# zzuiekongning/MGDT-YOLO

Hardware: AMD Instinct MI355X
Metric: images/sec @640x640 bs=32 per GPU, detection forward + NMS (whole job: 1 GPU(s)) (higher is better)
Workload: dtype bf16; 1 GPU; mspa_c2f_gd_yolov8-n (MSPA-C2f + GD neck + Detect, nc=80) 640x640 inference, batch 32/GPU: forward + decode + NMS(conf 0.25, iou 0.7), hipGraph replay, 4 batches in flight (one captured graph per resident batch, replayed round-robin on 4 streams); global_batch=32, parallelism=replicas x1 (batch-sharded, no data-path collective), rccl_ranks=1, input=bfloat16 NCHW images, 8 different batches resident in HBM (600 MiB) cycled, detections_last_step=9600, weights=seeded random init (no checkpoints offline), batches_in_flight=4

## Files before the change

### include/mgdt.h

```cpp
#ifndef MGDT_H
#define MGDT_H
#include <stddef.h>
#include <stdint.h>

#ifdef __cplusplus
extern "C" {
#endif

typedef void* mgdt_stream;

typedef enum { MGDT_OK = 0, MGDT_BAD_SHAPE = -1, MGDT_BAD_DTYPE = -2, MGDT_LAUNCH_FAIL = -3, MGDT_BAD_ARG = -4,
               MGDT_WORKSPACE = -5 } mgdt_status;
typedef enum { MGDT_F32 = 0, MGDT_BF16 = 1, MGDT_U8 = 2  } mgdt_dtype;
typedef enum { MGDT_ACT_NONE = 0, MGDT_ACT_SILU = 1, MGDT_ACT_RELU = 2, MGDT_ACT_GELU = 3 } mgdt_act;

typedef struct {
  void* p;
  int32_t n, h, w, c;
  int64_t sn, sh, sw, sc;
} mgdt_view;

const char* mgdt_last_error(void);
const char* mgdt_version(void);

size_t mgdt_conv_packed_bytes(int cin, int cout, int k, int dtype);
int mgdt_conv_pack(const float* w_oihw, const float* conv_bias, const float* bn_gamma, const float* bn_beta,
                   const float* bn_mean, const float* bn_var, float bn_eps, int cin, int cout, int k, int dtype,
                   void* packed_out, float* bias_out, mgdt_stream s);
int mgdt_conv_pack_dgrad(const float* w_oihw, int cin, int cout, int k, int phase, int dtype, void* packed_out, float* bias_out, mgdt_stream s);
typedef struct mgdt_pack_desc {
  const float* w; const float* conv_bias; const float* bn_gamma; const float* bn_beta; const float* bn_mean; const float* bn_var;
  float bn_eps; int32_t cin, cout, k, dtype, mode;
  void* packed; float* bias_out;
} mgdt_pack_desc;
int mgdt_conv_pack_batch(const mgdt_pack_desc* descs, int n, mgdt_stream s);

int mgdt_conv2d_fwd(const mgdt_view* x, const mgdt_view* x2, const float* in_scale, const float* in_shift,
                    const void* packed_w, const float* bias, int k, int stride, int act, const mgdt_view* r1,
                    const mgdt_view* r2, const mgdt_view* y, int dtype, mgdt_stream s);
size_t mgdt_conv_packed_bytes_fp8(int cin, int cout, int k);
int mgdt_conv_pack_fp8(const float* w_oihw, const float* conv_bias, const float* bn_gamma, const float* bn_beta, const float* bn_mean,
                       const float* bn_var, float bn_eps, int cin, int cout, int k, float x_qscale, void* packed_out, float* bias_out,
                       float* oscale_out, mgdt_stream s);
int mgdt_conv2d_fp8_fwd(const mgdt_view* x, const mgdt_view* x2, const float* in_scale, const float* in_shift, const void* packed_w,
                        const float* bias, const float* oscale, float x_qscale, int k, int stride, int act, const mgdt_view* r1,
                        const mgdt_view* r2, const mgdt_view* y, mgdt_stream s);
enum { MGDT_ROUTE_X2 = 1, MGDT_ROUTE_IN_SCALE = 2, MGDT_ROUTE_IN_SHIFT = 4, MGDT_ROUTE_R1 = 8, MGDT_ROUTE_R2 = 16, MGDT_ROUTE_FP8 = 32 };
enum { MGDT_ROUTE_IGEMM = 0, MGDT_ROUTE_LDS3X3 = 1 };
typedef struct {
  int32_t family, nchunks, waves, lds_bytes;
  int32_t NT, MT, D, extra, nseg, seg_chunks, gx, gy, numTiles, ragged;
  int32_t NBW, tile_rows, ncg, nwg, ntiles;
} mgdt_conv_route;
int mgdt_conv2d_route(const mgdt_view* x, const mgdt_view* y, int k, int stride, int dtype, int flags, int act, mgdt_conv_route* out);
int mgdt_conv2d_phase_fwd(const mgdt_view* x, const void* packed_w, const float* bias, int phase, const mgdt_view* r1, const mgdt_view* r2,
                          const mgdt_view* y, int dtype, mgdt_stream s);

size_t mgdt_cnx_mlp_packed_bytes(int c, int dtype);
int mgdt_cnx_mlp_pack(const float* w1, const float* b1, const float* w2, const float* b2, int c, void* packed, int dtype, mgdt_stream s);
size_t mgdt_cnx_mlp_workspace_bytes(int n, int h, int w, int c);
int mgdt_cnx_mlp_fwd(const mgdt_view* t, const mgdt_view* res, const void* packed, const float* gamma, const float* beta, void* ws,
                     const mgdt_view* y, int dtype, mgdt_stream s);

int mgdt_cnx_block_supported(int n, int h, int w, int c, int dtype);
size_t mgdt_cnx_block_workspace_bytes(int n, int h, int w, int c);
int mgdt_cnx_block_geometry(int h, int w, int c, int* out);
int mgdt_cnx_block_fwd(const mgdt_view* x, const float* dw_w49c, const float* dw_b, const float* ln_w, const float* ln_b, float eps, const void* packed,
                       const float* gamma, const float* beta, const void* tail_w, const float* tail_b, int tail_act, void* ws, size_t ws_bytes,
                       const mgdt_view* y, int dtype, mgdt_stream s);

size_t mgdt_stem2_packed_bytes(void);
int mgdt_stem2_pack(const float* w_folded, void* packed, mgdt_stream s);
int mgdt_stem2_fwd(const mgdt_view* x, int x_dtype, const void* packed0, const float* bias0, const void* packed1, const float* bias1,
                   const mgdt_view* y, mgdt_stream s);
int mgdt_stem2_geometry(int n, int h, int w, int cu_count, int* out);
int mgdt_stem2_route(const mgdt_view* x, int x_dtype, const mgdt_view* y, int cu_count, int* out);

int mgdt_detect_tail_supported(int c2, int c3, int nc, int reg_max, int dtype);
int mgdt_detect_tail_fwd(const mgdt_view* tb, const mgdt_view* tc, const void* wb, const float* bb, const void* wc, const float* bc, int nc,
                         float stride, int a_off, int a_total, const mgdt_view* feat, float* y, unsigned long long* best_keys,
                         const void* wb3, const float* bb3, mgdt_stream s);
int mgdt_detect_tail_aug_fwd(const mgdt_view* tb, const mgdt_view* tc, const void* wb, const float* bb, const void* wc, const float* bc, int nc,
                             float stride, int a_off, int a_total, const mgdt_view* feat, float* y, unsigned long long* best_keys,
                             const void* wb3, const float* bb3, float aug_scale, int aug_flip, float aug_img_w, mgdt_stream s);

// ... 251 lines not shown
```

### mgdt_yolo_amd/_lib.py

```python
import ctypes as C
import os

_HERE = os.path.dirname(os.path.abspath(__file__))
LIB_PATH = os.environ.get('MGDT_LIB') or os.path.join(_HERE, 'csrc', 'libmgdt_hip.so')

F32, BF16 = 0, 1
ACT_NONE, ACT_SILU, ACT_RELU, ACT_GELU = 0, 1, 2, 3
SPR_SPLITS = 16
GRN_SPLITS = 8


class View(C.Structure):
    _fields_ = [('p', C.c_void_p), ('n', C.c_int32), ('h', C.c_int32), ('w', C.c_int32), ('c', C.c_int32),
                ('sn', C.c_int64), ('sh', C.c_int64), ('sw', C.c_int64), ('sc', C.c_int64)]


VP = C.POINTER(View)
_vp, _i, _f, _sz, _l = C.c_void_p, C.c_int, C.c_float, C.c_size_t, C.c_long

class PackDesc(C.Structure):
    _fields_ = [('w', C.c_void_p), ('conv_bias', C.c_void_p), ('bn_gamma', C.c_void_p), ('bn_beta', C.c_void_p), ('bn_mean', C.c_void_p), ('bn_var', C.c_void_p),
                ('bn_eps', C.c_float), ('cin', C.c_int32), ('cout', C.c_int32), ('k', C.c_int32), ('dtype', C.c_int32), ('mode', C.c_int32),
                ('packed', C.c_void_p), ('bias_out', C.c_void_p)]


class WgradFinalDesc(C.Structure):
    _fields_ = [('partial', C.c_void_p), ('dw', C.c_void_p), ('n', C.c_long), ('nsplit', C.c_int32), ('accumulate', C.c_int32)]


class ConvRoute(C.Structure):
    _fields_ = [(n, C.c_int32) for n in ('family', 'nchunks', 'waves', 'lds_bytes', 'NT', 'MT', 'D', 'extra', 'nseg', 'seg_chunks', 'gx', 'gy', 'numTiles',
                                         'ragged', 'NBW', 'tile_rows', 'ncg', 'nwg', 'ntiles')]


ROUTE_X2, ROUTE_IN_SCALE, ROUTE_IN_SHIFT, ROUTE_R1, ROUTE_R2, ROUTE_FP8 = 1, 2, 4, 8, 16, 32
ROUTE_IGEMM, ROUTE_LDS3X3 = 0, 1
DIRECT_STEM, DIRECT_GENERIC, DIRECT_REFUSED = 0, 1, 2

PROTOTYPES = {
    'mgdt_last_error': (C.c_char_p, []),
    'mgdt_version': (C.c_char_p, []),
    'mgdt_conv_packed_bytes': (_sz, [_i, _i, _i, _i]),
    'mgdt_conv_pack': (_i, [_vp, _vp, _vp, _vp, _vp, _vp, _f, _i, _i, _i, _i, _vp, _vp, _vp]),
    'mgdt_conv2d_fwd': (_i, [VP, VP, _vp, _vp, _vp, _vp, _i, _i, _i, VP, VP, VP, _i, _vp]),
    'mgdt_conv_packed_bytes_fp8': (_sz, [_i, _i, _i]),
    'mgdt_conv_pack_fp8': (_i, [_vp, _vp, _vp, _vp, _vp, _vp, _f, _i, _i, _i, _f, _vp, _vp, _vp, _vp]),
    'mgdt_conv2d_fp8_fwd': (_i, [VP, VP, _vp, _vp, _vp, _vp, _vp, _f, _i, _i, _i, VP, VP, VP, _vp]),
    'mgdt_conv2d_route': (_i, [VP, VP, _i, _i, _i, _i, _i, C.POINTER(ConvRoute)]),
    'mgdt_conv_pack_batch': (_i, [_vp, _i, _vp]),
    'mgdt_conv2d_phase_fwd': (_i, [VP, _vp, _vp, _i, VP, VP, VP, _i, _vp]),
    'mgdt_conv_wgrad_splits': (_i, [_i, _i, _i]),
    'mgdt_wgrad_final_batch': (_i, [_vp, _i, _vp]),
    'mgdt_conv_pack_dgrad': (_i, [_vp, _i, _i, _i, _i, _i, _vp, _vp, _vp]),
    'mgdt_conv_pack_direct': (_i, [_vp, _vp, _vp, _vp, _vp, _vp, _f, _i, _i, _i, _vp, _vp, _vp]),
    'mgdt_conv2d_direct_fwd': (_i, [VP, _i, _vp, _vp, _i, _i, _i, _i, VP, _i, _vp]),
    'mgdt_conv2d_direct_route': (_i, [VP, _i, VP, _i, _i, _i, _i, C.POINTER(C.c_int)]),
    'mgdt_spr_pool_fwd': (_i, [VP, _vp, _i, _vp]),
    'mgdt_spr_attn_fwd': (_i, [_vp, _vp, _vp, _vp, _vp, _i, _i, _i, _i, _i, _i, _vp, _vp]),
    'mgdt_scale_channels_fwd': (_i, [VP, _vp, VP, _i, _vp]),
    'mgdt_sppf_pool_fwd': (_i, [VP, VP, VP, VP, _i, _vp]),
    'mgdt_adaptive_avgpool_fwd': (_i, [VP, VP, _i, _vp]),
    'mgdt_bilinear_fwd': (_i, [VP, VP, _i, _vp]),
    'mgdt_nearest_fwd': (_i, [VP, VP, _i, _vp]),
    'mgdt_copy_fwd': (_i, [VP, _i, VP, _i, _vp]),
    'mgdt_image_pad4_fwd': (_i, [VP, _i, VP, _i, _vp]),
    'mgdt_dwconv7_ln_fwd': (_i, [VP, _vp, _vp, _vp, _vp, _f, VP, _i, _vp]),
    'mgdt_cnx_mlp_packed_bytes': (_sz, [_i, _i]),
    'mgdt_cnx_mlp_pack': (_i, [_vp, _vp, _vp, _vp, _i, _vp, _i, _vp]),
    'mgdt_cnx_mlp_workspace_bytes': (_sz, [_i, _i, _i, _i]),
# ... 152 lines not shown
```

### mgdt_yolo_amd/csrc/common.h

```cpp
#pragma once
#include <atomic>
#include <hip/hip_runtime.h>
#include <stdint.h>
#include <stdio.h>
#include <string.h>

#include "../../include/mgdt.h"

typedef __bf16 bf16;
typedef __attribute__((ext_vector_type(8))) __bf16 bf16x8;
typedef __attribute__((ext_vector_type(4))) __bf16 bf16x4;
typedef __attribute__((ext_vector_type(4))) float f32x4;

#define MGDT_WAVE 64
#define POSE_MAX_NK 240

void mgdt_set_error(const char* fmt, ...);
#define MGDT_FAIL(code, ...)        \
  do {                              \
    mgdt_set_error(__VA_ARGS__);    \
    return (code);                  \
  } while (0)
#define MGDT_CHECK_LAUNCH(name)                                                   \
  do {                                                                            \
    hipError_t e_ = hipGetLastError();                                            \
    if (e_ != hipSuccess) MGDT_FAIL(MGDT_LAUNCH_FAIL, "%s: %s", name, hipGetErrorString(e_)); \
  } while (0)

static inline bool view_ok(const mgdt_view* v) { return v && v->p && v->n > 0 && v->h > 0 && v->w > 0 && v->c > 0; }
static inline bool view_nhwc(const mgdt_view* v) { return v->sc == 1; }
static inline int cdiv(long a, long b) { return (int)((a + b - 1) / b); }
static inline size_t dtype_size(int dt) { return dt == MGDT_BF16 ? 2 : 4; }

struct C3Plan { int NBW, MT, waves, ncg, nwg, tiles_x, tiles_per_img, ntiles, XP; size_t lds; long extx, exty; };

template <typename T> __device__ __forceinline__ float ldf(const T* p);
template <> __device__ __forceinline__ float ldf<float>(const float* p) { return *p; }
template <> __device__ __forceinline__ float ldf<bf16>(const bf16* p) { return (float)*p; }
template <typename T> __device__ __forceinline__ void stf(T* p, float v);
template <> __device__ __forceinline__ void stf<float>(float* p, float v) { *p = v; }
template <> __device__ __forceinline__ void stf<bf16>(bf16* p, float v) { *p = (bf16)v; }

template <typename T> __device__ __forceinline__ void store4(T* p, f32x4 v);
template <> __device__ __forceinline__ void store4<float>(float* p, f32x4 v) { *(f32x4*)p = v; }
template <> __device__ __forceinline__ void store4<bf16>(bf16* p, f32x4 v) {
  bf16x4 o;
#pragma unroll
  for (int i = 0; i < 4; ++i) o[i] = (bf16)v[i];
  *(bf16x4*)p = o;
}
template <typename T> __device__ __forceinline__ f32x4 load4(const T* p);
template <> __device__ __forceinline__ f32x4 load4<float>(const float* p) { return *(const f32x4*)p; }
template <> __device__ __forceinline__ f32x4 load4<bf16>(const bf16* p) {
  bf16x4 o = *(const bf16x4*)p;
  return f32x4{(float)o[0], (float)o[1], (float)o[2], (float)o[3]};
}


__device__ __forceinline__ float fast_sigmoid(float v) {
  return __builtin_amdgcn_rcpf(1.0f + __builtin_amdgcn_exp2f(-1.4426950408889634f * v));
}

__device__ __forceinline__ f32x4 mma_q8(long w, long p, f32x4 acc) {
  return __builtin_amdgcn_mfma_f32_16x16x32_fp8_fp8(w, p, acc, 0, 0, 0);
}
__device__ __forceinline__ long quant8(bf16x8 v, float xq) {
  typedef __attribute__((ext_vector_type(4))) unsigned int u32x4;
// ... 49 lines not shown
```

### mgdt_yolo_amd/csrc/conv_igemm.hip

```cpp
#include "conv_igemm_kernel.h"

struct FoldArgs { const float *cb, *g, *b, *mu, *var; float eps; int cout_real, cpad; float* bias_out; };
template <typename T>
__global__ void pack_kernel(const float* __restrict__ w, const float* __restrict__ scale, int Cin, int Cout, int KS,
                            int CP, int nchunks, int NTtot, T* __restrict__ out, int dgrad = 0, FoldArgs fa = FoldArgs{}) {
  constexpr int PE = Piece<T>::PE;
  long total = (long)nchunks * NTtot * 64 * PE;
  if (fa.bias_out && blockIdx.x == 0)
    for (int c = threadIdx.x; c < fa.cpad; c += blockDim.x) {
      float bo = 0.f;
      if (c < fa.cout_real) {
        if (fa.g) {
          const float s = fa.g[c] / sqrtf(fa.eps + fa.var[c]);
          bo = fa.b[c] - fa.g[c] * fa.mu[c] / sqrtf(fa.var[c] + fa.eps);
          if (fa.cb) bo += s * fa.cb[c];
        } else if (fa.cb) {
          bo = fa.cb[c];
        }
      }
      fa.bias_out[c] = bo;
    }
  for (long i = blockIdx.x * (long)blockDim.x + threadIdx.x; i < total; i += (long)gridDim.x * blockDim.x) {
    int j = (int)(i % PE);
    long t = i / PE;
// ... 252 lines not shown
  hipStream_t st = (hipStream_t)s;
  for (int dtype : {MGDT_F32, MGDT_BF16}) {
    PackJobs jobs;
    int m = 0;
    auto flush = [&]() {
      if (!m) return;
      for (int q = m; q < PACK_BATCH; ++q) { jobs.j[q] = jobs.j[0]; jobs.j[q].nchunks = 0; jobs.j[q].fa.bias_out = nullptr; }
      if (dtype == MGDT_F32) pack_batch_kernel<float><<<dim3(32, m), 256, 0, st>>>(jobs);
      else pack_batch_kernel<bf16><<<dim3(32, m), 256, 0, st>>>(jobs);
      m = 0;
    };
    for (int i = 0; i < n; ++i) {
      const mgdt_pack_desc& e = d[i];
      if (e.dtype != dtype) continue;
      if (!e.w || !e.packed || !e.bias_out) MGDT_FAIL(MGDT_BAD_ARG, "conv_pack_batch: descriptor %d has a null pointer", i);
      if (e.mode < 0 || e.mode > 5 || (e.mode >= 2 && e.k != 3)) MGDT_FAIL(MGDT_BAD_SHAPE, "conv_pack_batch: descriptor %d mode %d", i, e.mode);
      PackJob& J = jobs.j[m++];
      const int gi = e.mode == 0 ? e.cin : e.cout, go = e.mode == 0 ? e.cout : e.cin;
      conv_geometry(gi, go, e.k, dtype, &J.CP, &J.nchunks, &J.NTtot, e.mode >= 2 ? phase_ntaps(e.mode) : 0);
      J.w = e.w; J.Cin = gi; J.Cout = go; J.KS = e.k; J.dgrad = e.mode; J.out = e.packed;
      J.fa = e.mode == 0 ? FoldArgs{e.conv_bias, e.bn_gamma, e.bn_beta, e.bn_mean, e.bn_var, e.bn_eps, go, J.NTtot * 16, e.bias_out}
                         : FoldArgs{nullptr, nullptr, nullptr, nullptr, nullptr, 0.f, go, J.NTtot * 16, e.bias_out};
      if (m == PACK_BATCH) flush();
    }
    flush();
  }
  MGDT_CHECK_LAUNCH("conv_pack_batch");
  return MGDT_OK;
}

bool mgdt_conv3x3_lds_plan(const mgdt_view* x, const mgdt_view* y, int act, int CP, int nchunks, int NTtot, bool q8, int stride, C3Plan* p);
bool mgdt_conv3x3_lds_launch(const mgdt_view* x, const mgdt_view* y, const void* packed_w, const float* bias, int act, int CP, int nchunks, int NTtot, hipStream_t st,
                             const float* q8_oscale, float q8_xq, int stride);

template <typename T, int NT, int MT, bool Q8>
int launch_igemm(const ConvArgs& a, const IgemmPlan& p, hipStream_t st);

template <typename T>
static int dispatch_igemm(const ConvArgs& a, const IgemmPlan& p, hipStream_t st) {
  const int NT = p.NT, MT = p.MT;
#define CASE(nt, mt) \
  if (NT == nt && MT == mt) return launch_igemm<T, nt, mt, false>(a, p, st);
  CASE(1, 2) CASE(1, 4) CASE(2, 2) CASE(3, 2) CASE(4, 2) CASE(5, 2) CASE(6, 2) CASE(8, 2)
#undef CASE
  MGDT_FAIL(MGDT_BAD_SHAPE, "conv2d: no kernel for NT=%d MT=%d", NT, MT);
}

static int dispatch_igemm_q8(const ConvArgs& a, const IgemmPlan& p, hipStream_t st) {
  const int NT = p.NT;
#define CASE(nt) \
  if (NT == nt) return launch_igemm<bf16, nt, 2, true>(a, p, st);
  CASE(1) CASE(2) CASE(3) CASE(4) CASE(5) CASE(6) CASE(8)
#undef CASE
  MGDT_FAIL(MGDT_BAD_SHAPE, "conv2d_fp8: no kernel for NT=%d", NT);
}

static int conv_check_shapes(const mgdt_view* x, const mgdt_view* y, int k, int stride, int dtype, int* Ho_, int* Wo_) {
  if (dtype != MGDT_F32 && dtype != MGDT_BF16) MGDT_FAIL(MGDT_BAD_DTYPE, "conv2d: dtype %d", dtype);
  if ((k != 1 && k != 3) || (stride != 1 && stride != 2)) MGDT_FAIL(MGDT_BAD_SHAPE, "conv2d: k=%d stride=%d unsupported", k, stride);
  const int pe = piece_elems(dtype);
  const int pad = k / 2;
  const int Ho = (x->h + 2 * pad - k) / stride + 1, Wo = (x->w + 2 * pad - k) / stride + 1;
  if (y->n != x->n || y->h != Ho || y->w != Wo) MGDT_FAIL(MGDT_BAD_SHAPE, "conv2d: y is %dx%dx%d, expected %dx%dx%d", y->n, y->h, y->w, x->n, Ho, Wo);
  if (x->c % pe || y->c % 4) MGDT_FAIL(MGDT_BAD_SHAPE, "conv2d: cin=%d must be a multiple of %d and cout=%d of 4", x->c, pe, y->c);
  *Ho_ = Ho; *Wo_ = Wo;
  return MGDT_OK;
// ... 14 lines not shown
  int MT = 2;
  if (!q8 && NT == 1 && NTtot == 1) { const char* e = getenv("MGDT_CONV_MT1"); MT = e && atoi(e) == 4 ? 4 : 2; }
  int waves = 8;
  auto wgs = [&](int nt, int wv) { return (long)cdiv(M, 16 * wv * MT) * (NTtot / nt); };
  {
    const char* e = getenv("MGDT_CONV_MINWG");
    const int minwg = e ? atoi(e) : 128;
    while (wgs(NT, waves) < minwg && NT > 1 && NT % 2 == 0) NT /= 2;
  }
  {
    static const bool tail_split = getenv("MGDT_CONV_TAIL_SPLIT") != nullptr;
    const long w0 = wgs(NT, waves);
    if (tail_split && w0 > 768 && w0 <= 960 && NT % 2 == 0) NT /= 2;
  }
  {
    const char* e;
    if ((e = getenv("MGDT_CONV_WAVES"))) waves = std::min(8, std::max(1, atoi(e)));
  }
  p->numTiles = cdiv(M, 16 * waves * MT);
  p->T8 = cdiv(p->numTiles, 8);
  p->tab_bytes = (nchunks + 3) / 4 * 4 * 4 * 16;
  size_t panel = (size_t)nchunks * NT * WB;
  if (panel <= (size_t)LDS_PANEL_KIB * 1024) { p->seg_chunks = nchunks; p->nseg = 1; }
  else { p->seg_chunks = 64; p->nseg = cdiv(nchunks, p->seg_chunks); }
  p->lds = p->tab_bytes + (size_t)(q8 ? 2 : 1) * NT * 16 * sizeof(float) + (size_t)p->seg_chunks * NT * WB;
  int gcap = waves == 8 ? 256 : 1024;
  { const char* e = getenv("MGDT_CONV_GCAP"); if (e) gcap = atoi(e); }
  if (p->lds > 160 * 1024) MGDT_FAIL(MGDT_BAD_SHAPE, "conv2d: %zu bytes of LDS for NT=%d, %d chunks", p->lds, NT, p->seg_chunks);
  p->gx = std::min(8 * p->T8, gcap); p->gy = NTtot / NT;
  p->NT = NT; p->MT = MT; p->waves = waves;
  p->D = nchunks >= 3 ? 4 : 2;
  p->extra = extra;
  return MGDT_OK;
}

static int conv2d_fwd_impl(const mgdt_view* x, const mgdt_view* x2, const float* in_scale, const float* in_shift,
                           const void* packed_w, const float* bias, int k, int stride, int act, const mgdt_view* r1,
                           const mgdt_view* r2, const mgdt_view* y, int dtype, int tapmode, mgdt_stream s,
                           const float* q8_oscale = nullptr, float q8_xq = 1.f);
extern "C" int mgdt_conv2d_fwd(const mgdt_view* x, const mgdt_view* x2, const float* in_scale, const float* in_shift,
                               const void* packed_w, const float* bias, int k, int stride, int act, const mgdt_view* r1,
                               const mgdt_view* r2, const mgdt_view* y, int dtype, mgdt_stream s) {
  return conv2d_fwd_impl(x, x2, in_scale, in_shift, packed_w, bias, k, stride, act, r1, r2, y, dtype, 0, s);
}
extern "C" int mgdt_conv2d_phase_fwd(const mgdt_view* x, const void* packed_w, const float* bias, int phase, const mgdt_view* r1, const mgdt_view* r2,
                                     const mgdt_view* y, int dtype, mgdt_stream s) {
  if (phase < 0 || phase > 3) MGDT_FAIL(MGDT_BAD_ARG, "conv2d_phase: phase %d", phase);
  return conv2d_fwd_impl(x, nullptr, nullptr, nullptr, packed_w, bias, 3, 1, MGDT_ACT_NONE, r1, r2, y, dtype, 2 + phase, s);
}
extern "C" int mgdt_conv2d_fp8_fwd(const mgdt_view* x, const mgdt_view* x2, const float* in_scale, const float* in_shift,
                                   const void* packed_w, const float* bias, const float* oscale, float x_qscale, int k, int stride, int act,
                                   const mgdt_view* r1, const mgdt_view* r2, const mgdt_view* y, mgdt_stream s) {
  if (!oscale) MGDT_FAIL(MGDT_BAD_ARG, "conv2d_fp8: null oscale");
  if (!(x_qscale > 0.f) || !(x_qscale < 3.0e38f)) MGDT_FAIL(MGDT_BAD_ARG, "conv2d_fp8: x_qscale must be a positive finite number");
  return conv2d_fwd_impl(x, x2, in_scale, in_shift, packed_w, bias, k, stride, act, r1, r2, y, MGDT_BF16, 0, s, oscale, x_qscale);
}
static int conv2d_fwd_impl(const mgdt_view* x, const mgdt_view* x2, const float* in_scale, const float* in_shift,
                           const void* packed_w, const float* bias, int k, int stride, int act, const mgdt_view* r1,
                           const mgdt_view* r2, const mgdt_view* y, int dtype, int tapmode, mgdt_stream s,
                           const float* q8_oscale, float q8_xq) {
  const bool q8 = q8_oscale != nullptr;
  if (!view_ok(x) || !view_ok(y) || !packed_w || !bias) MGDT_FAIL(MGDT_BAD_ARG, "conv2d: null/empty view or weights");
  int Ho, Wo;
  if (int rc = conv_check_shapes(x, y, k, stride, dtype, &Ho, &Wo)) return rc;
  const int pe = piece_elems(dtype);
  const int pad = k / 2;
// ... 5 lines not shown
    if (rr && rr->p && (rr->n != y->n || rr->h != Ho || rr->w != Wo || rr->c != y->c || !aligned(rr, 4)))
      MGDT_FAIL(MGDT_BAD_SHAPE, "conv2d: residual must match y");

  ConvArgs a;
  memset(&a, 0, sizeof(a));
  const long sz = (long)dtype_size(dtype);
  auto extent = [&](const mgdt_view* v) { return ((long)(v->n - 1) * v->sn + (long)(v->h - 1) * v->sh + (long)(v->w - 1) * v->sw + v->c) * sz; };
  bool fits = true;
  auto bind = [&](const mgdt_view* v, const char** p, int* sn, int* sh, int* sw, uint32_t* bytes) {
    if (!v || !v->p) return;
    if (extent(v) >= 0x7fffffffL || v->sh * sz >= (1L << 23) || v->sw * sz >= (1L << 23)) { fits = false; return; }
    *p = (const char*)v->p; *sn = (int)(v->sn * sz); *sh = (int)(v->sh * sz); *sw = (int)(v->sw * sz); *bytes = (uint32_t)extent(v);
  };
  const char* yp = nullptr;
  bind(x, &a.x, &a.xsn, &a.xsh, &a.xsw, &a.x_bytes);
  bind(x2, &a.x2, &a.x2sn, &a.x2sh, &a.x2sw, &a.x2_bytes);
  bind(y, &yp, &a.ysn, &a.ysh, &a.ysw, &a.y_bytes);
  bind(r1, &a.r1, &a.r1sn, &a.r1sh, &a.r1sw, &a.r1_bytes);
  bind(r2, &a.r2, &a.r2sn, &a.r2sh, &a.r2sw, &a.r2_bytes);
  if (!fits) MGDT_FAIL(MGDT_BAD_SHAPE, "conv2d: a view spans >= 2 GiB or has a row stride >= 8 MiB");
  a.y = (char*)yp;
  a.in_scale = in_scale; a.in_shift = in_shift;
  a.wpk = (const char*)packed_w; a.bias = bias;
  a.oscale = q8_oscale; a.xq = q8_xq;
  a.N = x->n; a.H = x->h; a.W = x->w; a.Cin = x->c; a.Ho = Ho; a.Wo = Wo; a.Cout = y->c;
  a.KS = k; a.stride = stride; a.pad = pad; a.act = act;
  a.ntaps = tapmode >= 2 ? phase_ntaps(tapmode) : k * k;
  a.taplist = phase_taplist(tapmode, k);
  conv_geometry(a.Cin, a.Cout, k, dtype, &a.CP, &a.nchunks, &a.NTtot, tapmode >= 2 ? a.ntaps : 0);
  long M = (long)a.N * Ho * Wo;
  if (M > 0x7fffffffL - (1 << 20)) MGDT_FAIL(MGDT_BAD_SHAPE, "conv2d: problem too large");
  a.M = (int)M; a.HoWo = Ho * Wo;
  a.fd_howo = make_fastdiv((uint32_t)a.HoWo); a.fd_wo = make_fastdiv((uint32_t)Wo);
  if (conv_lds_candidate(tapmode, dtype, k, x2 && x2->p, in_scale, in_shift, r1 && r1->p, r2 && r2->p) &&
      mgdt_conv3x3_lds_launch(x, y, packed_w, bias, act, a.CP, a.nchunks, a.NTtot, (hipStream_t)s, q8_oscale, q8_xq, stride)) {
    MGDT_CHECK_LAUNCH("conv2d(3x3 lds)");
    return MGDT_OK;
  }

  IgemmPlan pl;
  if (int rc = igemm_plan(a.nchunks, a.NTtot, M, q8, a.x2 || a.in_scale || a.in_shift, &pl)) return rc;
  a.numTiles = pl.numTiles; a.T8 = pl.T8; a.tab_bytes = pl.tab_bytes; a.seg_chunks = pl.seg_chunks; a.nseg = pl.nseg;
  hipStream_t st = (hipStream_t)s;
  if (q8) return dispatch_igemm_q8(a, pl, st);
  if (dtype == MGDT_F32) return dispatch_igemm<float>(a, pl, st);
  return dispatch_igemm<bf16>(a, pl, st);
}

extern "C" int mgdt_conv2d_route(const mgdt_view* x, const mgdt_view* y, int k, int stride, int dtype, int flags, int act, mgdt_conv_route* out) {
  if (!x || !y || !out || x->n <= 0 || x->h <= 0 || x->w <= 0 || x->c <= 0 || y->c <= 0) MGDT_FAIL(MGDT_BAD_ARG, "conv2d_route: null/empty view");
  const bool q8 = flags & MGDT_ROUTE_FP8;
  if (q8 && dtype != MGDT_BF16) MGDT_FAIL(MGDT_BAD_DTYPE, "conv2d_route: the fp8 kernels take bf16 views");
  int Ho, Wo;
  if (int rc = conv_check_shapes(x, y, k, stride, dtype, &Ho, &Wo)) return rc;
  mgdt_view xv = *x, yv = *y;
  xv.p = yv.p = nullptr;
  if (!conv_view_aligned(&xv, piece_elems(dtype), dtype) || !conv_view_aligned(&yv, 4, dtype))
    MGDT_FAIL(MGDT_BAD_SHAPE, "conv2d: x/y must be NHWC views (sc==1) with 16-byte aligned pieces");
  int CP, nchunks, NTtot;
  conv_geometry(x->c, y->c, k, dtype, &CP, &nchunks, &NTtot);
  const long M = (long)x->n * Ho * Wo;
  if (M > 0x7fffffffL - (1 << 20)) MGDT_FAIL(MGDT_BAD_SHAPE, "conv2d: problem too large");
  memset(out, 0, sizeof(*out));
  out->nchunks = nchunks;
  C3Plan c3;
  if (conv_lds_candidate(0, dtype, k, flags & MGDT_ROUTE_X2, flags & MGDT_ROUTE_IN_SCALE, flags & MGDT_ROUTE_IN_SHIFT, flags & MGDT_ROUTE_R1, flags & MGDT_ROUTE_R2) &&
      mgdt_conv3x3_lds_plan(&xv, &yv, act, CP, nchunks, NTtot, q8, stride, &c3)) {
    out->family = MGDT_ROUTE_LDS3X3;
    out->NBW = c3.NBW; out->tile_rows = 4 * c3.MT; out->ncg = c3.ncg; out->nwg = c3.nwg; out->ntiles = c3.ntiles; out->waves = c3.waves;
    out->lds_bytes = (int)c3.lds;
    return MGDT_OK;
  }
  IgemmPlan pl;
  if (int rc = igemm_plan(nchunks, NTtot, M, q8, flags & (MGDT_ROUTE_X2 | MGDT_ROUTE_IN_SCALE | MGDT_ROUTE_IN_SHIFT), &pl)) return rc;
  out->family = MGDT_ROUTE_IGEMM;
  out->NT = pl.NT; out->MT = pl.MT; out->D = pl.D; out->extra = pl.extra; out->nseg = pl.nseg; out->seg_chunks = pl.seg_chunks; out->waves = pl.waves;
  out->gx = pl.gx; out->gy = pl.gy; out->numTiles = pl.numTiles; out->lds_bytes = (int)pl.lds;
  out->ragged = NTtot * 16 > y->c;
  return MGDT_OK;
}
```

### mgdt_yolo_amd/ops.py

```python
import ctypes as C
import os

import torch

from . import _lib as L
from ._lib import ACT_GELU, ACT_NONE, ACT_RELU, ACT_SILU, BF16, F32, View

U8 = 2
_DT = {torch.float32: F32, torch.bfloat16: BF16}


def dtype_code(dt):
    try:
        return _DT[dt]
    except KeyError:
        raise RuntimeError(f'mgdt_yolo_amd computes in float32 or bfloat16, not {dt}') from None


def _need_gpu(t):
    if not t.is_cuda:
        raise RuntimeError('mgdt_yolo_amd runs on MI355X (HIP) only: got a CPU tensor and there is no CPU/PyTorch fallback')


_PROF = None
# ... 229 lines not shown
    b, _, h, w = x.shape
    ho, wo = conv_out_hw(h, w, pk.k, stride)
    if out is None:
        out = new_act(b, pk.cout, ho, wo, pk.dtype, x.device)
    if _PROF is not None:
        es = out.element_size()
        _META['conv2d_direct_fwd' if pk.direct else 'conv2d_fwd'] = dict(
            shape=(b, pk.cin, h, w, pk.cout, pk.k, stride), flops=2.0 * b * ho * wo * pk.cout * pk.cin // pk.groups * pk.k * pk.k,
            bytes=float(b * h * w * pk.cin * x.element_size() + b * ho * wo * pk.cout * es + pk.w.numel() * pk.w.element_size()))
    if pk.direct:
        if x2 is not None or r1 is not None or r2 is not None or in_scale is not None or in_shift is not None:
            raise RuntimeError('direct convolution path has no fused extras')
        _launch('conv2d_direct_fwd', 'mgdt_conv2d_direct_fwd', vp(x), U8 if x.dtype == torch.uint8 else dtype_code(x.dtype), ptr(pk.w), ptr(pk.bias), pk.k, stride, pk.groups, act,
                                           vp(out), dtype_code(out.dtype), stream())
    else:
        _same(x, x2, r1, r2, out)
        if x.dtype != pk.dtype:
            raise RuntimeError(f'conv2d: the weights are packed for {pk.dtype}, the input is {x.dtype}')
        _launch('conv2d_fwd', 'mgdt_conv2d_fwd', vp(x), vp(x2), ptr(in_scale), ptr(in_shift), ptr(pk.w), ptr(pk.bias), pk.k, stride, act,
                                    vp(r1), vp(r2), vp(out), dtype_code(pk.dtype), stream())
    return out


def conv2d_route(x, y, k, stride, dtype=None, act=ACT_SILU, x2=False, in_scale=False, in_shift=False, r1=False, r2=False, fp8=False):
    def shape_view(t):
        b, c, h, w = t.shape
        sn, sc, sh, sw = t.stride()
        return View(None, b, h, w, c, sn, sh, sw, sc)
    flags = sum(f for on, f in ((x2, L.ROUTE_X2), (in_scale, L.ROUTE_IN_SCALE), (in_shift, L.ROUTE_IN_SHIFT), (r1, L.ROUTE_R1), (r2, L.ROUTE_R2),
                                (fp8, L.ROUTE_FP8)) if on)
    r = L.ConvRoute()
    L.check(L.lib().mgdt_conv2d_route(C.byref(shape_view(x)), C.byref(shape_view(y)), k, stride, dtype_code(dtype or x.dtype), flags, act, C.byref(r)),
            'conv2d_route')
    keys = (('NT', 'MT', 'D', 'extra', 'nseg', 'seg_chunks', 'gx', 'gy', 'numTiles', 'ragged') if r.family == L.ROUTE_IGEMM
            else ('NBW', 'tile_rows', 'ncg', 'nwg', 'ntiles'))
    out = {'family': 'igemm' if r.family == L.ROUTE_IGEMM else 'lds3x3'}
    out.update((n, getattr(r, n)) for n in keys + ('waves', 'nchunks', 'lds_bytes'))
    return out


def _route_view(t):
    b, c, h, w = t.shape
    sn, sc, sh, sw = t.stride()
    p = 4096 + t.storage_offset() * t.element_size() if t.device.type == 'meta' else t.data_ptr()
    return View(p, b, h, w, c, sn, sh, sw, sc)


def _image_code(dt):
    return dt if isinstance(dt, int) else (U8 if dt == torch.uint8 else dtype_code(dt))


def conv2d_direct_route(x, y, k, stride, groups=1, x_dtype=None, dtype=None):
    out = (C.c_int * 4)()
    L.check(L.lib().mgdt_conv2d_direct_route(C.byref(_route_view(x)), _image_code(x.dtype if x_dtype is None else x_dtype), C.byref(_route_view(y)),
                                             _image_code(y.dtype if dtype is None else dtype), int(k), int(stride), int(groups), out), 'conv2d_direct_route')
    return dict(family=('stem', 'generic', 'refused')[out[0]], gx=out[1], gy=out[2], status=out[3])


def spr_attention(x, fc1_w, fc1_b, fc2_w, fc2_b, groups, softmax=True):
    b, c, h, w = x.shape
    lib = L.lib()
    part = torch.empty(b * L.SPR_SPLITS * c * 5, dtype=torch.float32, device=x.device)
    _launch('spr_pool_fwd', 'mgdt_spr_pool_fwd', vp(x), ptr(part), dtype_code(x.dtype), stream())
    attn = torch.empty(b, c, dtype=torch.float32, device=x.device)
    _launch('spr_attn_fwd', 'mgdt_spr_attn_fwd', ptr(part), ptr(fc1_w), ptr(fc1_b), ptr(fc2_w), ptr(fc2_b), b, c, groups, h, w, int(bool(softmax)),
            ptr(attn), stream())
    return attn


# ... 1618 lines not shown
```

Measured before the change: 41430 images/sec.

## Add LDS-banded streaming kernel for stride-2 3x3 convs that underfill the GPU

Adds a new conv path for stride-2 3x3 bf16 convolutions that the LDS3x3 path rejects and whose implicit-GEMM grid is small. Each workgroup loads a band of input rows (5 output rows) into LDS once, then streams weight chunks through an 8-deep register ring feeding MFMA 16x16x32. The goal is to reuse input from LDS and pipeline weight loads better than the igemm fallback for the low-resolution downsampling convs. It is on by default for workgroup counts between 16 and 256, can be turned off with an env var, and adds optional timestamp instrumentation.

Measured after the change: 41730 images/sec (median of 6 runs). Within noise of the previous version (+0.7%).

```diff
diff --git a/include/mgdt.h b/include/mgdt.h
--- a/include/mgdt.h
+++ b/include/mgdt.h
@@ -46,11 +46,12 @@
                         const float* bias, const float* oscale, float x_qscale, int k, int stride, int act, const mgdt_view* r1,
                         const mgdt_view* r2, const mgdt_view* y, mgdt_stream s);
 enum { MGDT_ROUTE_X2 = 1, MGDT_ROUTE_IN_SCALE = 2, MGDT_ROUTE_IN_SHIFT = 4, MGDT_ROUTE_R1 = 8, MGDT_ROUTE_R2 = 16, MGDT_ROUTE_FP8 = 32 };
-enum { MGDT_ROUTE_IGEMM = 0, MGDT_ROUTE_LDS3X3 = 1 };
+enum { MGDT_ROUTE_IGEMM = 0, MGDT_ROUTE_LDS3X3 = 1, MGDT_ROUTE_S2STREAM = 2 };
 typedef struct {
   int32_t family, nchunks, waves, lds_bytes;
   int32_t NT, MT, D, extra, nseg, seg_chunks, gx, gy, numTiles, ragged;
   int32_t NBW, tile_rows, ncg, nwg, ntiles;
+  int32_t band_rows, nbands, ngroups;
 } mgdt_conv_route;
 int mgdt_conv2d_route(const mgdt_view* x, const mgdt_view* y, int k, int stride, int dtype, int flags, int act, mgdt_conv_route* out);
 int mgdt_conv2d_phase_fwd(const mgdt_view* x, const void* packed_w, const float* bias, int phase, const mgdt_view* r1, const mgdt_view* r2,
diff --git a/mgdt_yolo_amd/_lib.py b/mgdt_yolo_amd/_lib.py
--- a/mgdt_yolo_amd/_lib.py
+++ b/mgdt_yolo_amd/_lib.py
@@ -30,11 +30,11 @@
 
 class ConvRoute(C.Structure):
     _fields_ = [(n, C.c_int32) for n in ('family', 'nchunks', 'waves', 'lds_bytes', 'NT', 'MT', 'D', 'extra', 'nseg', 'seg_chunks', 'gx', 'gy', 'numTiles',
-                                         'ragged', 'NBW', 'tile_rows', 'ncg', 'nwg', 'ntiles')]
+                                         'ragged', 'NBW', 'tile_rows', 'ncg', 'nwg', 'ntiles', 'band_rows', 'nbands', 'ngroups')]
 
 
 ROUTE_X2, ROUTE_IN_SCALE, ROUTE_IN_SHIFT, ROUTE_R1, ROUTE_R2, ROUTE_FP8 = 1, 2, 4, 8, 16, 32
-ROUTE_IGEMM, ROUTE_LDS3X3 = 0, 1
+ROUTE_IGEMM, ROUTE_LDS3X3, ROUTE_S2STREAM = 0, 1, 2
 DIRECT_STEM, DIRECT_GENERIC, DIRECT_REFUSED = 0, 1, 2
 
 PROTOTYPES = {
diff --git a/mgdt_yolo_amd/csrc/common.h b/mgdt_yolo_amd/csrc/common.h
--- a/mgdt_yolo_amd/csrc/common.h
+++ b/mgdt_yolo_amd/csrc/common.h
@@ -33,6 +33,7 @@
 static inline size_t dtype_size(int dt) { return dt == MGDT_BF16 ? 2 : 4; }
 
 struct C3Plan { int NBW, MT, waves, ncg, nwg, tiles_x, tiles_per_img, ntiles, XP; size_t lds; long extx, exty; };
+struct S2SPlan { int TH, NBW, waves, ncg, nbands, ngroups, nwg, RW, XP; size_t lds; long extx, exty; };
 
 template <typename T> __device__ __forceinline__ float ldf(const T* p);
 template <> __device__ __forceinline__ float ldf<float>(const float* p) { return *p; }
diff --git a/mgdt_yolo_amd/csrc/conv_igemm.hip b/mgdt_yolo_amd/csrc/conv_igemm.hip
--- a/mgdt_yolo_amd/csrc/conv_igemm.hip
+++ b/mgdt_yolo_amd/csrc/conv_igemm.hip
@@ -308,6 +308,9 @@
 bool mgdt_conv3x3_lds_plan(const mgdt_view* x, const mgdt_view* y, int act, int CP, int nchunks, int NTtot, bool q8, int stride, C3Plan* p);
 bool mgdt_conv3x3_lds_launch(const mgdt_view* x, const mgdt_view* y, const void* packed_w, const float* bias, int act, int CP, int nchunks, int NTtot, hipStream_t st,
                              const float* q8_oscale, float q8_xq, int stride);
+bool mgdt_conv_s2s_plan(const mgdt_view* x, const mgdt_view* y, int act, int CP, int nchunks, int NTtot, S2SPlan* p);
+int mgdt_conv_s2s_launch(const mgdt_view* x, const mgdt_view* y, const void* packed_w, const float* bias, int act, int CP, int nchunks, int NTtot, const S2SPlan& pl,
+                         hipStream_t st);
 
 template <typename T, int NT, int MT, bool Q8>
 int launch_igemm(const ConvArgs& a, const IgemmPlan& p, hipStream_t st);
@@ -388,6 +391,14 @@
   p->D = nchunks >= 3 ? 4 : 2;
   p->extra = extra;
   return MGDT_OK;
+}
+
+static bool s2s_plan(bool cand, const mgdt_view* x, const mgdt_view* y, int stride, bool q8, int act, int CP, int nchunks, int NTtot, const IgemmPlan& ig, S2SPlan* p) {
+  int mode = 1;
+  { const char* e = getenv("MGDT_CONV_S2STREAM"); if (e) mode = atoi(e); }
+  if (!mode || !cand || stride != 2 || q8 || ig.numTiles > ig.gx) return false;
+  if (!mgdt_conv_s2s_plan(x, y, act, CP, nchunks, NTtot, p)) return false;
+  return mode >= 2 || (p->nwg >= 16 && p->nwg <= 256);
 }
 
 static int conv2d_fwd_impl(const mgdt_view* x, const mgdt_view* x2, const float* in_scale, const float* in_shift,
@@ -459,14 +470,17 @@
   if (M > 0x7fffffffL - (1 << 20)) MGDT_FAIL(MGDT_BAD_SHAPE, "conv2d: problem too large");
   a.M = (int)M; a.HoWo = Ho * Wo;
   a.fd_howo = make_fastdiv((uint32_t)a.HoWo); a.fd_wo = make_fastdiv((uint32_t)Wo);
-  if (conv_lds_candidate(tapmode, dtype, k, x2 && x2->p, in_scale, in_shift, r1 && r1->p, r2 && r2->p) &&
-      mgdt_conv3x3_lds_launch(x, y, packed_w, bias, act, a.CP, a.nchunks, a.NTtot, (hipStream_t)s, q8_oscale, q8_xq, stride)) {
+  const bool cand = conv_lds_candidate(tapmode, dtype, k, x2 && x2->p, in_scale, in_shift, r1 && r1->p, r2 && r2->p);
+  if (cand && mgdt_conv3x3_lds_launch(x, y, packed_w, bias, act, a.CP, a.nchunks, a.NTtot, (hipStream_t)s, q8_oscale, q8_xq, stride)) {
     MGDT_CHECK_LAUNCH("conv2d(3x3 lds)");
     return MGDT_OK;
   }
 
   IgemmPlan pl;
   if (int rc = igemm_plan(a.nchunks, a.NTtot, M, q8, a.x2 || a.in_scale || a.in_shift, &pl)) return rc;
+  S2SPlan sp;
+  if (s2s_plan(cand, x, y, stride, q8, act, a.CP, a.nchunks, a.NTtot, pl, &sp))
+    return mgdt_conv_s2s_launch(x, y, packed_w, bias, act, a.CP, a.nchunks, a.NTtot, sp, (hipStream_t)s);
   a.numTiles = pl.numTiles; a.T8 = pl.T8; a.tab_bytes = pl.tab_bytes; a.seg_chunks = pl.seg_chunks; a.nseg = pl.nseg;
   hipStream_t st = (hipStream_t)s;
   if (q8) return dispatch_igemm_q8(a, pl, st);
@@ -491,8 +505,8 @@
   memset(out, 0, sizeof(*out));
   out->nchunks = nchunks;
   C3Plan c3;
-  if (conv_lds_candidate(0, dtype, k, flags & MGDT_ROUTE_X2, flags & MGDT_ROUTE_IN_SCALE, flags & MGDT_ROUTE_IN_SHIFT, flags & MGDT_ROUTE_R1, flags & MGDT_ROUTE_R2) &&
-      mgdt_conv3x3_lds_plan(&xv, &yv, act, CP, nchunks, NTtot, q8, stride, &c3)) {
+  const bool cand = conv_lds_candidate(0, dtype, k, flags & MGDT_ROUTE_X2, flags & MGDT_ROUTE_IN_SCALE, flags & MGDT_ROUTE_IN_SHIFT, flags & MGDT_ROUTE_R1, flags & MGDT_ROUTE_R2);
+  if (cand && mgdt_conv3x3_lds_plan(&xv, &yv, act, CP, nchunks, NTtot, q8, stride, &c3)) {
     out->family = MGDT_ROUTE_LDS3X3;
     out->NBW = c3.NBW; out->tile_rows = 4 * c3.MT; out->ncg = c3.ncg; out->nwg = c3.nwg; out->ntiles = c3.ntiles; out->waves = c3.waves;
     out->lds_bytes = (int)c3.lds;
@@ -500,6 +514,13 @@
   }
   IgemmPlan pl;
   if (int rc = igemm_plan(nchunks, NTtot, M, q8, flags & (MGDT_ROUTE_X2 | MGDT_ROUTE_IN_SCALE | MGDT_ROUTE_IN_SHIFT), &pl)) return rc;
+  S2SPlan sp;
+  if (s2s_plan(cand, &xv, &yv, stride, q8, act, CP, nchunks, NTtot, pl, &sp)) {
+    out->family = MGDT_ROUTE_S2STREAM;
+    out->NBW = sp.NBW; out->ncg = sp.ncg; out->nwg = sp.nwg; out->waves = sp.waves; out->band_rows = sp.TH; out->nbands = sp.nbands; out->ngroups = sp.ngroups;
+    out->lds_bytes = (int)sp.lds;
+    return MGDT_OK;
+  }
   out->family = MGDT_ROUTE_IGEMM;
   out->NT = pl.NT; out->MT = pl.MT; out->D = pl.D; out->extra = pl.extra; out->nseg = pl.nseg; out->seg_chunks = pl.seg_chunks; out->waves = pl.waves;
   out->gx = pl.gx; out->gy = pl.gy; out->numTiles = pl.numTiles; out->lds_bytes = (int)pl.lds;
diff --git a/mgdt_yolo_amd/csrc/conv_s2_stream.hip b/mgdt_yolo_amd/csrc/conv_s2_stream.hip
--- /dev/null
+++ b/mgdt_yolo_amd/csrc/conv_s2_stream.hip
@@ -0,0 +1,234 @@
+#include <vector>
+
+#include "conv_igemm_kernel.h"
+
+#define S2S_TH 5
+#define S2S_NBW 8
+#define S2S_MAXDBG 4096
+
+struct S2SArgs {
+  const char* x; int xsn, xsh, xsw; uint32_t x_bytes;
+  char* y; int ysn, ysh, ysw; uint32_t y_bytes;
+  const char* wpk; const float* bias;
+  int H, W, Ho, Wo, Cout, CP, CPQ, nchunks, NTtot, ncg, nbands, nwg, RW, XP, nitems;
+  FastDiv fd_cp, fd_rw, fd_wo, fd_ncg, fd_nb;
+  unsigned long long* dbg;
+};
+
+template <int ACT>
+__global__ __launch_bounds__(512, 1) void conv_s2_stream_kernel(const S2SArgs a) {
+  constexpr int NTHR = 512, MT = 4, NBH = 2, RING = 8, L = RING - 1, MAXI = 16;
+  static_assert(RING % 2 == 0, "the B double buffer follows the ring slot's parity");
+  extern __shared__ __attribute__((aligned(16))) char xs[];
+  const int tid = threadIdx.x, lane = tid & 63, r = lane & 15, g = lane >> 4;
+  const int wave = __builtin_amdgcn_readfirstlane(tid >> 6);
+  const int per = gridDim.x >> 3;
+  const int id = (blockIdx.x & 7) * per + (blockIdx.x >> 3);
+  if (id >= a.nwg) return;
+  const int t = (int)fdiv((uint32_t)id, a.fd_ncg), cg = id - t * a.ncg;
+  const int n = (int)fdiv((uint32_t)t, a.fd_nb), band = t - n * a.nbands;
+  const int oy0 = band * S2S_TH, rows = min(S2S_TH, a.Ho - oy0), np = rows * a.Wo, ngroups = (np + 15) >> 4;
+  const int iy0 = 2 * oy0 - 1;
+  const __amdgpu_buffer_rsrc_t xrs = __builtin_amdgcn_make_buffer_rsrc((void*)a.x, 0, a.x_bytes, 0x00020000);
+  const __amdgpu_buffer_rsrc_t yrs = __builtin_amdgcn_make_buffer_rsrc((void*)a.y, 0, a.y_bytes, 0x00020000);
+  unsigned long long T0 = 0, T1 = 0, T2 = 0, T3 = 0;
+  if (a.dbg) T0 = __builtin_amdgcn_s_memrealtime();
+
+  const int nbw0 = cg * S2S_NBW + (wave & 3) * NBH, ph = wave >> 2;
+  int nbc[NBH];
+#pragma unroll
+  for (int bw = 0; bw < NBH; ++bw) nbc[bw] = min(nbw0 + bw, a.NTtot - 1);
+  const char* const wlane = a.wpk + (size_t)lane * 16;
+  const size_t wstep = (size_t)a.NTtot * 1024;
+  bf16x8 A[RING][NBH];
+  auto load_a = [&](int kc, auto stag) __attribute__((always_inline)) {
+    constexpr int s = decltype(stag)::value;
+    const char* p = wlane + (size_t)min(kc, a.nchunks - 1) * wstep;
+#pragma unroll
+    for (int bw = 0; bw < NBH; ++bw) A[s][bw] = *(const bf16x8*)(p + (size_t)nbc[bw] * 1024);
+  };
+  auto prefetch_a = [&]() __attribute__((always_inline)) {
+    load_a(0, std::integral_constant<int, 0>{}); load_a(1, std::integral_constant<int, 1>{}); load_a(2, std::integral_constant<int, 2>{});
+    load_a(3, std::integral_constant<int, 3>{}); load_a(4, std::integral_constant<int, 4>{}); load_a(5, std::integral_constant<int, 5>{});
+    load_a(6, std::integral_constant<int, 6>{});
+  };
+
+  for (int base = 0; base < a.nitems; base += MAXI * NTHR) {
+    uint4 st[MAXI];
+#pragma unroll
+    for (int u = 0; u < MAXI; ++u) {
+      const int it = base + tid + u * NTHR;
+      const int pix = (int)fdiv((uint32_t)it, a.fd_cp), c8 = it - pix * a.CP;
+      const int py = (int)fdiv((uint32_t)pix, a.fd_rw), px = pix - py * a.RW;
+      const int iy = iy0 + py, ix = px - 1;
+      const bool ok = it < a.nitems && (unsigned)iy < (unsigned)a.H && (unsigned)ix < (unsigned)a.W;
+      st[u] = __builtin_bit_cast(uint4, __builtin_amdgcn_raw_buffer_load_b128(xrs, ok ? (uint32_t)(n * a.xsn + iy * a.xsh + ix * a.xsw + c8 * 16) : (uint32_t)MGDT_OOB, 0, 0));
+    }
+    if (base == 0) {
+      prefetch_a();
+      if (a.dbg) T1 = __builtin_amdgcn_s_memrealtime();
+    }
+#pragma unroll
+    for (int u = 0; u < MAXI; ++u) {
+      const int it = base + tid + u * NTHR;
+      const int pix = (int)fdiv((uint32_t)it, a.fd_cp), c8 = it - pix * a.CP;
+      if (it < a.nitems) *(uint4*)(xs + (size_t)pix * a.XP + c8 * 16) = st[u];
+    }
+  }
+  __syncthreads();
+  if (a.dbg) T2 = __builtin_amdgcn_s_memrealtime();
+  if (nbw0 >= a.NTtot) return;
+
+  f32x4 bias[NBH];
+#pragma unroll
+  for (int bw = 0; bw < NBH; ++bw) bias[bw] = *(const f32x4*)(a.bias + nbc[bw] * 16 + 4 * g);
+
+  bool first = true;
+  for (int gs = ph * MT; gs < ngroups; gs += 2 * MT) {
+    if (!first) prefetch_a();
+    first = false;
+    int bbase[MT], yo[MT];
+#pragma unroll
+    for (int m = 0; m < MT; ++m) {
+      const int q = (gs + m) * 16 + r;
+      const bool pv = q < np;
+      const int qq = pv ? q : 0;
+      const int oyl = (int)fdiv((uint32_t)qq, a.fd_wo), ox = qq - oyl * a.Wo;
+      bbase[m] = (2 * oyl * a.RW + 2 * ox) * a.XP + g * 16;
+      yo[m] = pv ? n * a.ysn + (oy0 + oyl) * a.ysh + ox * a.ysw : MGDT_OOB;
+    }
+    f32x4 acc[NBH][MT];
+#pragma unroll
+    for (int bw = 0; bw < NBH; ++bw)
+#pragma unroll
+      for (int m = 0; m < MT; ++m) acc[bw][m] = bias[bw];
+
+    bf16x8 B[2][MT];
+    int tapn = 0, cqn = 0, koffn = 0;
+    auto load_b = [&](auto btag) __attribute__((always_inline)) {
+      constexpr int b = decltype(btag)::value;
+#pragma unroll
+      for (int m = 0; m < MT; ++m) B[b][m] = *(const bf16x8*)(xs + bbase[m] + koffn);
+      koffn += 64;
+      if (++cqn == a.CPQ) {
+        cqn = 0; ++tapn;
+        const int ty = (tapn * 11) >> 5, tx = tapn - 3 * ty;
+        koffn = tapn < 9 ? (ty * a.RW + tx) * a.XP : 0;
+      }
+    };
+    auto step = [&](int j, auto stag) __attribute__((always_inline)) {
+      constexpr int s = decltype(stag)::value;
+      load_a(j + L, std::integral_constant<int, (s + L) % RING>{});
+      load_b(std::integral_constant<int, (s + 1) & 1>{});
+#pragma unroll
+      for (int bw = 0; bw < NBH; ++bw)
+#pragma unroll
+        for (int m = 0; m < MT; ++m) acc[bw][m] = __builtin_amdgcn_mfma_f32_16x16x32_bf16(A[s][bw], B[s & 1][m], acc[bw][m], 0, 0, 0);
+    };
+    load_b(std::integral_constant<int, 0>{});
+    int j = 0;
+    for (; j + RING <= a.nchunks; j += RING) {
+      step(j, std::integral_constant<int, 0>{}); step(j + 1, std::integral_constant<int, 1>{}); step(j + 2, std::integral_constant<int, 2>{});
+      step(j + 3, std::integral_constant<int, 3>{}); step(j + 4, std::integral_constant<int, 4>{}); step(j + 5, std::integral_constant<int, 5>{});
+      step(j + 6, std::integral_constant<int, 6>{}); step(j + 7, std::integral_constant<int, 7>{});
+    }
+    const int rem = a.nchunks - j;
+    if (rem > 0) step(j, std::integral_constant<int, 0>{});
+    if (rem > 1) step(j + 1, std::integral_constant<int, 1>{});
+    if (rem > 2) step(j + 2, std::integral_constant<int, 2>{});
+    if (rem > 3) step(j + 3, std::integral_constant<int, 3>{});
+    if (rem > 4) step(j + 4, std::integral_constant<int, 4>{});
+    if (rem > 5) step(j + 5, std::integral_constant<int, 5>{});
+    if (rem > 6) step(j + 6, std::integral_constant<int, 6>{});
+    if (a.dbg) T3 = __builtin_amdgcn_s_memrealtime();
+
+#pragma unroll
+    for (int m = 0; m < MT; ++m) {
+#pragma unroll
+      for (int bw = 0; bw < NBH; ++bw) {
+        const int co = (nbw0 + bw) * 16 + 4 * g;
+        f32x4 v = acc[bw][m];
+#pragma unroll
+        for (int e = 0; e < 4; ++e) {
+          if (ACT == MGDT_ACT_SILU) v[e] = v[e] * fast_sigmoid(v[e]);
+          else if (ACT == MGDT_ACT_RELU) v[e] = fmaxf(v[e], 0.f);
+        }
+        const int dead = co < a.Cout ? 0 : MGDT_OOB;
+        bstore4<bf16>(yrs, (uint32_t)(yo[m] | dead) + (uint32_t)(co * 2), v);
+      }
+    }
+  }
+  if (a.dbg && tid == 0 && id < S2S_MAXDBG) {
+    unsigned long long* d = a.dbg + (size_t)id * 5;
+    d[0] = T0; d[1] = T1; d[2] = T2; d[3] = T3; d[4] = __builtin_amdgcn_s_memrealtime();
+  }
+}
+
+bool mgdt_conv_s2s_plan(const mgdt_view* x, const mgdt_view* y, int act, int CP, int nchunks, int NTtot, S2SPlan* p) {
+  const int Cin = x->c, Cout = y->c;
+  if (Cin % 32 || Cin < 96 || Cout % 4 || (act != MGDT_ACT_SILU && act != MGDT_ACT_NONE && act != MGDT_ACT_RELU)) return false;
+  if (nchunks != 9 * (CP / 4)) return false;
+  p->extx = ((long)(x->n - 1) * x->sn + (long)(x->h - 1) * x->sh + (long)(x->w - 1) * x->sw + x->c) * 2;
+  p->exty = ((long)(y->n - 1) * y->sn + (long)(y->h - 1) * y->sh + (long)(y->w - 1) * y->sw + y->c) * 2;
+  if (p->extx >= 0x7fffffffL || p->exty >= 0x7fffffffL) return false;
+  p->TH = S2S_TH; p->NBW = S2S_NBW; p->waves = 8;
+  p->XP = Cin * 2 + 16;
+  p->RW = 2 * y->w + 1;
+  const long lds = (long)(2 * S2S_TH + 1) * p->RW * p->XP;
+  if (lds > 160 * 1024) return false;
+  p->lds = (size_t)lds;
+  p->ncg = cdiv(NTtot, S2S_NBW);
+  p->nbands = cdiv(y->h, S2S_TH);
+  p->ngroups = cdiv((long)std::min(S2S_TH, y->h) * y->w, 16);
+  const long nwg = (long)x->n * p->nbands * p->ncg;
+  if (nwg > (1 << 20)) return false;
+  p->nwg = (int)nwg;
+  return true;
+}
+
+int mgdt_conv_s2s_launch(const mgdt_view* x, const mgdt_view* y, const void* packed_w, const float* bias, int act, int CP, int nchunks, int NTtot, const S2SPlan& pl,
+                         hipStream_t st) {
+  S2SArgs a;
+  memset(&a, 0, sizeof(a));
+  a.x = (const char*)x->p; a.xsn = (int)(x->sn * 2); a.xsh = (int)(x->sh * 2); a.xsw = (int)(x->sw * 2); a.x_bytes = (uint32_t)pl.extx;
+  a.y = (char*)y->p; a.ysn = (int)(y->sn * 2); a.ysh = (int)(y->sh * 2); a.ysw = (int)(y->sw * 2); a.y_bytes = (uint32_t)pl.exty;
+  a.wpk = (const char*)packed_w; a.bias = bias;
+  a.H = x->h; a.W = x->w; a.Ho = y->h; a.Wo = y->w; a.Cout = y->c; a.CP = CP; a.CPQ = CP / 4; a.nchunks = nchunks; a.NTtot = NTtot;
+  a.ncg = pl.ncg; a.nbands = pl.nbands; a.nwg = pl.nwg; a.RW = pl.RW; a.XP = pl.XP;
+  a.nitems = (2 * S2S_TH + 1) * pl.RW * CP;
+  a.fd_cp = make_fastdiv((uint32_t)CP); a.fd_rw = make_fastdiv((uint32_t)pl.RW); a.fd_wo = make_fastdiv((uint32_t)a.Wo);
+  a.fd_ncg = make_fastdiv((uint32_t)pl.ncg); a.fd_nb = make_fastdiv((uint32_t)pl.nbands);
+  static unsigned long long* dbgbuf = nullptr;
+  const bool dbg = getenv("MGDT_S2S_DBG") != nullptr;
+  if (dbg && !dbgbuf) (void)hipMalloc((void**)&dbgbuf, S2S_MAXDBG * 5 * 8);
+  a.dbg = dbg ? dbgbuf : nullptr;
+  const int grid = cdiv(pl.nwg, 8) * 8;
+#define S2S_LAUNCH(ACTV)                                                                                                                          \
+  {                                                                                                                                               \
+    static std::atomic<bool> attr{false};                                                                                                         \
+    if (!attr) {                                                                                                                                  \
+      hipError_t e = hipFuncSetAttribute((const void*)conv_s2_stream_kernel<ACTV>, hipFuncAttributeMaxDynamicSharedMemorySize, 160 * 1024);       \
+      if (e != hipSuccess) MGDT_FAIL(MGDT_LAUNCH_FAIL, "conv2d(s2 stream): hipFuncSetAttribute: %s", hipGetErrorString(e));                       \
+      attr = true;                                                                                                                                \
+    }                                                                                                                                             \
+    conv_s2_stream_kernel<ACTV><<<grid, 512, pl.lds, st>>>(a);                                                                                    \
+  }
+  if (act == MGDT_ACT_SILU) S2S_LAUNCH(MGDT_ACT_SILU) else if (act == MGDT_ACT_RELU) S2S_LAUNCH(MGDT_ACT_RELU) else S2S_LAUNCH(MGDT_ACT_NONE)
+#undef S2S_LAUNCH
+  MGDT_CHECK_LAUNCH("conv2d(s2 stream)");
+  if (a.dbg) {
+    const int nd = std::min(pl.nwg, S2S_MAXDBG);
+    std::vector<unsigned long long> h((size_t)nd * 5);
+    (void)hipStreamSynchronize(st);
+    (void)hipMemcpy(h.data(), dbgbuf, h.size() * 8, hipMemcpyDeviceToHost);
+    unsigned long long t0 = ~0ull, t1 = 0; double rq = 0, rl = 0, mf = 0, ep = 0;
+    for (int i = 0; i < nd; ++i) {
+      const unsigned long long* d = &h[(size_t)i * 5];
+      t0 = std::min(t0, d[0]); t1 = std::max(t1, d[4]);
+      rq += d[1] - d[0]; rl += d[2] - d[1]; mf += d[3] - d[2]; ep += d[4] - d[3];
+    }
+    fprintf(stderr, "conv_s2_stream cin %d cout %d %dx%d: %d wgs, span %.1f us; wave 0 of a workgroup (us): region requested %.2f, region in LDS %.2f, mfma loop %.2f, epilogue %.2f\n",
+            x->c, y->c, x->h, x->w, pl.nwg, (t1 - t0) * 0.01, rq / nd * 0.01, rl / nd * 0.01, mf / nd * 0.01, ep / nd * 0.01);
+  }
+  return MGDT_OK;
+}
diff --git a/mgdt_yolo_amd/ops.py b/mgdt_yolo_amd/ops.py
--- a/mgdt_yolo_amd/ops.py
+++ b/mgdt_yolo_amd/ops.py
@@ -285,9 +285,10 @@
     r = L.ConvRoute()
     L.check(L.lib().mgdt_conv2d_route(C.byref(shape_view(x)), C.byref(shape_view(y)), k, stride, dtype_code(dtype or x.dtype), flags, act, C.byref(r)),
             'conv2d_route')
-    keys = (('NT', 'MT', 'D', 'extra', 'nseg', 'seg_chunks', 'gx', 'gy', 'numTiles', 'ragged') if r.family == L.ROUTE_IGEMM
-            else ('NBW', 'tile_rows', 'ncg', 'nwg', 'ntiles'))
-    out = {'family': 'igemm' if r.family == L.ROUTE_IGEMM else 'lds3x3'}
+    keys = {L.ROUTE_IGEMM: ('NT', 'MT', 'D', 'extra', 'nseg', 'seg_chunks', 'gx', 'gy', 'numTiles', 'ragged'),
+            L.ROUTE_LDS3X3: ('NBW', 'tile_rows', 'ncg', 'nwg', 'ntiles'),
+            L.ROUTE_S2STREAM: ('NBW', 'ncg', 'nwg', 'band_rows', 'nbands', 'ngroups')}[r.family]
+    out = {'family': {L.ROUTE_IGEMM: 'igemm', L.ROUTE_LDS3X3: 'lds3x3', L.ROUTE_S2STREAM: 's2stream'}[r.family]}
     out.update((n, getattr(r, n)) for n in keys + ('waves', 'nchunks', 'lds_bytes'))
     return out
 
```
